# shibatch/rectdetect

Measured on AMD Instinct MI355X. Metric: 1920x1080 frames/sec, higher is better.
Workload: dtype u8/i32/f32 (bit-exact integer + IEEE f32 stencil path)

## Files before the change

rectdetect_amd/csrc/rd_k_rect.hip:

```cpp
#include <stdlib.h>
#include "rd_device.h"
#include "rd_kernels.h"
#include "rd_tidy_tile.h"
#include "rd_poly_scratch.h"
#include "rd_post_core.h"
#include <atomic>

namespace {

using namespace rd;

inline int cdiv(int a, int b) { return (a + b - 1) / b; }
const dim3 block2(64, 4);
inline dim3 grid2(int iw, int ih) { return dim3(cdiv(iw, 64), cdiv(ih, 4)); }
inline int ew_grid(int n) { int g = cdiv(n, 256 * 4); return g < 1 ? 1 : (g > 4096 ? 4096 : g); }

#define RD_XY const int x = blockIdx.x * 64 + threadIdx.x, y = blockIdx.y * 4 + rd_ty()

typedef unsigned long long u64;
__device__ __forceinline__ bitrow row_m1(const u64 *__restrict__ plane, int wpr, int y, int k, int ih) {
  if (y < 0 || y >= ih) return br(0, 0);
  const u64 *r = plane + (size_t)y * wpr + k;
  const u64 W = k > 0 ? r[-1] : 0ull, C = r[0], E = k + 1 < wpr ? r[1] : 0ull;
  return br((W >> 63) | (C << 1), (C >> 63) | (E << 1));
// ... 151 lines not shown
  const int tx = threadIdx.x, wv = rd_ty(), tid = wv * 64 + tx;
  const int x0 = rd_b.x * 64, y0 = rd_b.y * BQ_ROWS;
  const int x = x0 + tx, r0 = 8 * wv;
  const unsigned pb = (unsigned)((y0 - 4 + r0) * iw + x);
  unsigned eh[8];
  uint32_t q[8], qh;
  const int sr = tid >> 3, sc = (tid & 7) + ((tid & 4) << 4);
  const bool interior = x0 >= 4 && y0 >= 4 && x0 + 68 <= iw && y0 + BQ_ROWS + 4 <= ih;
  if (interior) {
#pragma unroll
    for (int j = 0; j < 8; j++) {
      const unsigned a = pb + (unsigned)((j < BQ_HR - 56 || r0 + j < BQ_HR ? j : 0) * iw);
      q[j] = atu(in, a);
      eh[j] = atu(ext, a);
    }
    qh = atu(in, (unsigned)((y0 - 4) * iw + x0 - 4) + (unsigned)__umul24(sr < BQ_HR ? sr : 0, iw) + (unsigned)sc);
#pragma unroll
    for (int j = BQ_HR - 56; j < 8; j++) if (r0 + j >= BQ_HR) { q[j] = 0u; eh[j] = 0u; }
  } else {
    bool ok[8];
    const bool cx = x < iw;
#pragma unroll
    for (int j = 0; j < 8; j++) {
      const int r = r0 + j, y = y0 - 4 + r;
      ok[j] = r < BQ_HR && y >= 0 && y < ih && cx;
      const unsigned a = ok[j] ? pb + (unsigned)(j * iw) : 0u;
      q[j] = atu(in, a);
      eh[j] = atu(ext, a);
    }
    const int xx = x0 - 4 + sc, yy = y0 - 4 + sr;
    const bool okq = sr < BQ_HR && xx >= 0 && xx < iw && yy >= 0 && yy < ih;
    qh = atu(in, okq ? (unsigned)(yy * iw + xx) : 0u);
#pragma unroll
    for (int j = 0; j < 8; j++) if (!ok[j]) { q[j] = 0u; eh[j] = 0u; }
    if (!okq) qh = 0u;
  }
  if (tid < 64) { const unsigned w = (unsigned)((tid & 7) + (tid >> 3)); rwt[tid] = w >= 1 && w <= 10 ? ((1u << 19) + w - 1u) / w : 0u; }
  char *const plb = (char *)pl;
  const unsigned hb = (unsigned)((r0 * BQ_SW + tx + 4) * 8);
  u64 cell[8];
#pragma unroll
  for (int j = 0; j < 8; j++) {
    const uint32_t v = q[j];
    cell[j] = (u64)((v & 4095u) | ((v << 4) & 0x3ff0000u)) | ((u64)(v >> 22) << 32);
    if (j < BQ_HR - 56 || r0 + j < BQ_HR) *(u64 *)(plb + hb + (unsigned)(j * BQ_SW * 8)) = cell[j];
  }
  if (sr < BQ_HR) pl[sr * BQ_SW + sc] = (u64)((qh & 4095u) | ((qh << 4) & 0x3ff0000u)) | ((u64)(qh >> 22) << 32);
  __syncthreads();
  {
    u64 v[9];
    const unsigned b = (unsigned)(((tx < BQ_HR ? tx : BQ_HR - 1) * BQ_SW + 9 * wv) * 8);
#pragma unroll
    for (int j = 0; j < 9; j++) v[j] = *(const u64 *)(plb + b + (unsigned)(8 * j));
    u64 sum = v[0];
#pragma unroll
    for (int j = 1; j < 9; j++) sum += v[j];
    tot[wv * 64 + tx] = sum;
    __syncthreads();
    u64 off = 0, ts[7];
#pragma unroll
    for (int s2 = 0; s2 < 7; s2++) ts[s2] = s2 < wv ? tot[s2 * 64 + tx] : 0;
#pragma unroll
    for (int s2 = 0; s2 < 7; s2++) off += ts[s2];
    if (tx < BQ_HR) {
#pragma unroll
      for (int j = 0; j < 9; j++) { *(u64 *)(plb + b + (unsigned)(8 * j)) = off; off += v[j]; }
      if (wv == 7) *(u64 *)(plb + b + 72u) = off;
    }
  }
  __syncthreads();
  u64 o[8], osum = 0;
#pragma unroll
  for (int j0 = 0; j0 < 8; j0 += BQ_WB) {
    u64 hi[BQ_WB], lo[BQ_WB];
    unsigned rw[BQ_WB];
#pragma unroll
    for (int u = 0; u < BQ_WB; u++) {
      const int j = j0 + u;
      const unsigned e = eh[j];
      const unsigned c = hb + (unsigned)((j < BQ_HR - 56 || r0 + j < BQ_HR ? j : 0) * BQ_SW * 8);
      hi[u] = *(const u64 *)(plb + c + (e & 0x38u));
      lo[u] = *(const u64 *)(plb + c + 8u - ((e & 7u) << 3));
      rw[u] = *(const unsigned *)((const char *)rwt + ((e & 63u) << 2));
    }
#pragma unroll
    for (int u = 0; u < BQ_WB; u++) {
      const int j = j0 + u;
      const u64 a = hi[u] - lo[u] + cell[j];
      const unsigned ax = (unsigned)a, ay = (unsigned)(a >> 32);
      o[j] = (u64)(div_small_m(ax & 0xffffu, rw[u]) | (div_small_m(ax >> 16, rw[u]) << 16)) | ((u64)div_small_m(ay, rw[u]) << 32);
      osum += o[j];
    }
  }
  tot[wv * 64 + tx] = osum;
  __syncthreads();
  const unsigned vb = (unsigned)((r0 * 64 + tx) * 8);
  {
    u64 off = 0, ts[7];
#pragma unroll
    for (int s2 = 0; s2 < 7; s2++) ts[s2] = s2 < wv ? tot[s2 * 64 + tx] : 0;
#pragma unroll
    for (int s2 = 0; s2 < 7; s2++) off += ts[s2];
#pragma unroll
    for (int j = 0; j < 8; j++) { *(u64 *)(plb + vb + (unsigned)(j * 512)) = off; off += o[j]; }
  }
  __syncthreads();
  if (x >= iw) return;
#pragma unroll
  for (int j0 = 0; j0 < 8; j0 += BQ_WB) {
    u64 hi[BQ_WB], lo[BQ_WB];
    unsigned rw[BQ_WB];
#pragma unroll
    for (int u = 0; u < BQ_WB; u++) {
      const int j = j0 + u, r = r0 + j;
      if (r < 4 || r >= BQ_ROWS + 4 || y0 - 4 + r >= ih) continue;
      const unsigned e = eh[j];
      const unsigned c = vb + (unsigned)(j * 512);
      hi[u] = *(const u64 *)(plb + c + (e & 0xe00u));
      lo[u] = *(const u64 *)(plb + c + 512u - ((e & 0x1c0u) << 3));
      rw[u] = *(const unsigned *)((const char *)rwt + ((e >> 4) & 0xfcu));
    }
#pragma unroll
    for (int u = 0; u < BQ_WB; u++) {
      const int j = j0 + u, r = r0 + j;
      if (r < 4 || r >= BQ_ROWS + 4 || y0 - 4 + r >= ih) continue;
      const u64 a = hi[u] - lo[u] + o[j];
      const unsigned ax = (unsigned)a, ay = (unsigned)(a >> 32);
      atu(out, pb + (unsigned)(j * iw)) = div_small_m(ax & 0xffffu, rw[u]) | (div_small_m(ax >> 16, rw[u]) << 12) | (div_small_m(ay, rw[u]) << 22);
    }
  }
}

__device__ __forceinline__ uint32_t quantize_plab(uint32_t v, int n0, int n1, int n2) {
  float L, a, b;
  unpack_lab(v, L, a, b);
  return pack_lab(roundf(L * n0) / (float)n0, roundf(a * n1) / (float)n1, roundf(b * n2) / (float)n2);
}

__device__ __attribute__((aligned(16))) uint16_t g_quant24[4096 + 1024];
__global__ void k_quant24_lut() {
  const int i = blockIdx.x * blockDim.x + threadIdx.x;
  if (i < 4096) g_quant24[i] = (uint16_t)(quantize_plab((uint32_t)i, 24, 24, 24) & 4095u);
  else if (i < 5120) g_quant24[i] = (uint16_t)((quantize_plab((uint32_t)(i - 4096) << 12, 24, 24, 24) >> 12) & 1023u);
}

#ifndef DS_ROWS
#define DS_ROWS 30
#endif
#define DS_P 66
#define DS_R (DS_ROWS + 2)
#define DS_RW (DS_R / 4)
static_assert(DS_R % 4 == 0 && 2 * DS_R <= 256 && DS_R <= 64, "rows by four waves; one halo cell per thread; a list entry is row << 6 | column in 16 bits");
template <int QN>
__global__ __launch_bounds__(256) void k_despeckle(uint32_t *__restrict__ out, const uint32_t *__restrict__ in, const float *__restrict__ edge, int iw, int ih, size_t zs, int gdim) {
  const rd_tile rd_b = rd_block_tile(gdim);
  if (rd_b.x < 0) return;
  RD_ZSHIFTZ(rd_b.z, zs, out, in, edge);
  __shared__ uint32_t tq[DS_R * DS_P];
  __shared__ uint8_t tf[DS_R * DS_P];
  __shared__ uint16_t list[4][64 * DS_RW];
  __shared__ int nlist[4];
  __shared__ uint32_t qlut[QN == 24 ? 2560 : 1];
  const int tx = threadIdx.x, wv = rd_ty(), tid = wv * 64 + tx;
  const int x0 = rd_b.x * 64, y0 = rd_b.y * DS_ROWS;
  const bool colin = x0 + tx < iw;
  const unsigned cx = (unsigned)(x0 + (colin ? tx : 0));
  uint32_t v[DS_RW + 1];
  float e[DS_RW + 1];
#pragma unroll
  for (int k = 0; k < DS_RW; k++) {
    const int y = y0 - 1 + wv + 4 * k, yc = y < 0 ? 0 : (y >= ih ? ih - 1 : y);
    const unsigned a = (unsigned)(yc * iw) + cx;
    v[k] = atu(in, a);
    e[k] = atu(edge, a);
  }
  const int hs = tid >> 1, hc = (tid & 1) * (DS_P - 1);
  const int hx = x0 - 1 + hc, hy = y0 - 1 + hs;
  const bool hok = hs < DS_R && hx >= 0 && hx < iw && hy >= 0 && hy < ih;
  {
    const unsigned a = hok ? (unsigned)(hy * iw + hx) : 0u;
    v[DS_RW] = atu(in, a);
    e[DS_RW] = atu(edge, a);
  }
  if (QN == 24) {
    uint32_t w[10];
#pragma unroll
    for (int i = 0; i < 10; i++) w[i] = atu((const uint32_t *)g_quant24, (unsigned)(tid + 256 * i));
#pragma unroll
    for (int i = 0; i < 10; i++) qlut[tid + 256 * i] = w[i];
    __syncthreads();
  }
  auto quant = [&](uint32_t c) -> uint32_t {
    if (QN == 24) {
      const uint16_t *q16 = (const uint16_t *)qlut;
      return (uint32_t)q16[c & 4095u] | ((uint32_t)q16[4096 + ((c >> 12) & 1023u)] << 12) | ((uint32_t)q16[4096 + (c >> 22)] << 22);
    }
    return QN > 0 ? quantize_plab(c, QN, QN, QN) : c;
  };
#pragma unroll
  for (int k = 0; k <= DS_RW; k++) v[k] = quant(v[k]);
  int nhot = 0;
#pragma unroll
  for (int k = 0; k < DS_RW; k++) {
    const int s = wv + 4 * k, y = y0 - 1 + s;
    const bool ok = colin && y >= 0 && y < ih, mine = ok && s >= 1 && s <= DS_ROWS;
    const uint32_t qv = v[k];
    const bool hot = !(e[k] < 1e-6f), skip = e[k] >= 1e-6f;
    const int i = s * DS_P + tx + 1;
    tq[i] = qv;
    tf[i] = ok && !skip ? 0 : 1;
    if (mine && !hot) atu(out, (unsigned)(y * iw + x0 + tx)) = qv;
    const unsigned long long m = __builtin_amdgcn_ballot_w64(mine && hot);
    if (m) {
      if (mine && hot) list[wv][nhot + (int)__builtin_amdgcn_mbcnt_hi((unsigned)(m >> 32), __builtin_amdgcn_mbcnt_lo((unsigned)m, 0u))] = (uint16_t)((s << 6) | tx);
      nhot += __popcll(m);
    }
  }
  if (hs < DS_R) {
    const int i = hs * DS_P + hc;
    tq[i] = v[DS_RW];
    tf[i] = hok && !(e[DS_RW] >= 1e-6f) ? 0 : 1;
  }
  if (tx == 0) nlist[wv] = nhot;
  __syncthreads();
  const int n1 = nlist[0], n2 = n1 + nlist[1], n3 = n2 + nlist[2], n = n3 + nlist[3];
  for (int j = tid; j < n; j += 256) {
    const int w = (j >= n1) + (j >= n2) + (j >= n3);
    const int en = list[w][j - (w == 0 ? 0 : (w == 1 ? n1 : (w == 2 ? n2 : n3)))];
    const int s = en >> 6, c = en & 63;
    const int i = s * DS_P + c + 1;
    uint32_t r = tq[i];
    float dist = 1e+10f, l0, a0, b0;
    unpack_lab(r, l0, a0, b0);
#pragma unroll
    for (int k = 0; k < 9; k++) {
      const int q = i + (k / 3 - 1) * DS_P + k % 3 - 1;
      if (tf[q]) continue;
      float l1, a1, b1;
      const uint32_t v1 = tq[q];
      unpack_lab(v1, l1, a1, b1);
      const float dx = l1 - l0, dy = a1 - a0, dz = b1 - b0;
      const float d = sqrtf(dx * dx + dy * dy + dz * dz);
      if (d < dist) { r = v1; dist = d; }
    }
    atu(out, (unsigned)((y0 + s - 1) * iw + x0 + c)) = r;
  }
}

template <int DX>
__device__ __forceinline__ unsigned long long mm_shift(unsigned long long w0, unsigned long long w1, unsigned long long w2) {
  if (DX == 0) return w1;
  if (DX > 0) return (w1 >> DX) | (w2 << (64 - DX));
  return (w1 << -DX) | (w0 >> (64 + DX));
}
template <int DY, int LO, int HI, int DX = -8>
__device__ __forceinline__ unsigned long long mm_row(unsigned long long w0, unsigned long long w1, unsigned long long w2) {
  unsigned long long r = 0;
  if (DX * DX + DY * DY >= LO && DX * DX + DY * DY < HI) r = mm_shift<DX>(w0, w1, w2);
  if constexpr (DX < 8) r |= mm_row<DY, LO, HI, DX + 1>(w0, w1, w2);
  return r;
}
template <int DY>
__device__ __forceinline__ void mm_rows(const unsigned long long *sb, int r, unsigned long long &A, unsigned long long &B, unsigned long long &C) {
  const unsigned long long *row = sb + (r + 8 + DY) * 6;
  const unsigned long long a0 = row[0], a1 = row[1], a2 = row[2], e0 = row[3], e1 = row[4], e2 = row[5];
  constexpr int ADY = DY < 0 ? -DY : DY;
  if (ADY * ADY < 36) A |= mm_row<ADY, 16, 36>(a0, a1, a2);
  if (ADY * ADY < 64) B |= mm_row<ADY, 0, 64>(e0, e1, e2);
  if (ADY * ADY < 16) C |= mm_row<ADY, 0, 16>(a0 & ~e0, a1 & ~e1, a2 & ~e2);
  if constexpr (DY < 8) mm_rows<DY + 1>(sb, r, A, B, C);
}

#define MM_ROWS 64
__global__ __launch_bounds__(256) void k_mm_gather(unsigned long long *__restrict__ out, const unsigned long long *__restrict__ bits, int iw, int ih, int wpr, size_t zs) {
  RD_ZSHIFT(zs, out, bits);
  __shared__ unsigned long long sb[(MM_ROWS + 16) * 6];
  const int k = blockIdx.x;
  const int y0 = blockIdx.y * MM_ROWS;
  const int tid = rd_ty() * 64 + threadIdx.x;
  for (int t = tid; t < (MM_ROWS + 16) * 6; t += 256) {
    const int r = t / 6, j = t % 6;
    const int yy = y0 - 8 + r, kk = k - 1 + j % 3;
    unsigned long long v = 0ull;
    if (yy >= 0 && yy < ih && kk >= 0 && kk < wpr) v = bits[((size_t)yy * wpr + kk) * 2 + j / 3];
    sb[t] = v;
  }
  __syncthreads();
  if (tid < MM_ROWS && y0 + tid < ih) {
    unsigned long long A = 0, B = 0, C = 0;
    mm_rows<-8>(sb, tid, A, B, C);
    const int left = iw - 64 * k;
    out[(size_t)(y0 + tid) * wpr + k] = A & ~B & ~C & (left >= 64 ? ~0ull : ((1ull << left) - 1ull));
  }
}

#define RR_NFLAGS (RD_REGION_STATUS_AT + 32)
static_assert(RD_REGION_STATUS_AT >= RD_REGION_MAX_LAUNCHES && RR_NFLAGS <= 256, "k_region_init clears the flag words with one block of 256 threads");
#ifndef RI_ROWS
#define RI_ROWS 32
#endif
#define RI_H 10
#define RI_RW (64 + RI_H + 2)
#define RI_RH (RI_ROWS + RI_H + 2)
#define RI_NC (RI_RW * RI_RH)
__global__ __launch_bounds__(256) void k_region_init(int *__restrict__ A, int *__restrict__ B, u64 *__restrict__ allow, const int *__restrict__ pix, const u64 *__restrict__ mask,
                                                     const u64 *__restrict__ edge, int iw, int ih, int wpr, int *__restrict__ flags, int *__restrict__ size_out, size_t zs, int gdim) {
  const rd_tile rd_b = rd_block_tile(gdim);
  if (rd_b.x < 0) return;
  RD_ZSHIFTZ(rd_b.z, zs, A, B, allow, pix, mask, edge, flags, size_out);
  __shared__ u64 sm[(RI_ROWS + 2) * 2];
  __shared__ u64 se[(RI_ROWS + 3) * 3];
  __shared__ int col[RI_NC];
  __shared__ short lnk[RI_NC];
  __shared__ short prop[RI_NC];
  __shared__ unsigned char alw[RI_NC];
  const int tid = rd_ty() * 64 + threadIdx.x;
  if (rd_b.x == 0 && rd_b.y == 0 && tid < RR_NFLAGS) flags[tid] = tid == 0 ? 1 : 0;
  const int gx0 = rd_b.x * 64 - RI_H, gy0 = rd_b.y * RI_ROWS - RI_H;
  {
    constexpr int NR = (RI_RH + 3) / 4, NS = (RI_RH * 16 + 255) / 256;
    const int wv = rd_ty(), lx = threadIdx.x;
    int v[NR + NS];
    bool ok[NR + NS];
    u64 wm = 0, we = 0;
    bool okm = false, oke = false;
    {
      const int k = rd_b.x, yb0 = rd_b.y * RI_ROWS;
      { const int r = tid >> 1, kk = k + (tid & 1), yy = yb0 + r; okm = tid < (RI_ROWS + 2) * 2 && yy < ih && kk < wpr; wm = mask[okm ? (size_t)yy * wpr + kk : 0]; }
      { const int r = tid / 3, kk = k - 1 + tid % 3, yy = yb0 - 1 + r; oke = tid < (RI_ROWS + 3) * 3 && yy >= 0 && yy < ih && kk >= 0 && kk < wpr; we = edge[oke ? (size_t)yy * wpr + kk : 0]; }
    }
    const int gxl = gx0 + lx;
    const bool cok = gxl >= 0 && gxl < iw;
#pragma unroll
    for (int i = 0; i < NR; i++) {
      const int r = wv + 4 * i, gy = gy0 + r;
      ok[i] = r < RI_RH && gy >= 0 && gy < ih && cok;
      v[i] = atu(pix, ok[i] ? (unsigned)(gy * iw + gxl) : 0u);
    }
#pragma unroll
    for (int j = 0; j < NS; j++) {
      const int t = tid + 256 * j, r = t >> 4, c = 64 + (t & 15);
      const int gx = gx0 + c, gy = gy0 + r;
      ok[NR + j] = r < RI_RH && c < RI_RW && gx < iw && gy >= 0 && gy < ih;
      v[NR + j] = atu(pix, ok[NR + j] ? (unsigned)(gy * iw + gx) : 0u);
    }
#pragma unroll
    for (int i = 0; i < NR; i++) {
      const int r = wv + 4 * i;
      if (r < RI_RH) { col[r * RI_RW + lx] = v[i]; lnk[r * RI_RW + lx] = ok[i] ? 0 : -1; }
    }
#pragma unroll
    for (int j = 0; j < NS; j++) {
      const int t = tid + 256 * j, r = t >> 4, c = 64 + (t & 15);
      if (r < RI_RH && c < RI_RW) { col[r * RI_RW + c] = v[NR + j]; lnk[r * RI_RW + c] = ok[NR + j] ? 0 : -1; }
    }
    if (tid < (RI_ROWS + 2) * 2) sm[tid] = okm ? wm : 0ull;
    if (tid < (RI_ROWS + 3) * 3) se[tid] = oke ? we : 0ull;
  }
  constexpr int MW = 64 + 2, MH = RI_ROWS + 2, MN = MW * MH;
  __syncthreads();
  (void)MN;
  {
    auto cell = [&](int cy, int cx) {
      const int gx = gx0 + RI_H + cx, gy = gy0 + RI_H + cy;
      const unsigned mbit = (unsigned)(sm[cy * 2 + (cx >> 6)] >> (cx & 63)) & 1u, ebit = (unsigned)(se[(cy + 1) * 3 + 1 + (cx >> 6)] >> (cx & 63)) & 1u;
      alw[(RI_H + cy) * RI_RW + RI_H + cx] = (unsigned char)((gx < iw && gy < ih) ? (mbit | (ebit ? 0u : 2u)) : 0u);
    };
    for (int cy = rd_ty(); cy < MH; cy += 4) cell(cy, (int)threadIdx.x);
    if (tid < 2 * MH) cell(tid >> 1, 64 + (tid & 1));
    static_assert(MW == 66, "two columns beyond the lanes");
  }
  {
    auto cell = [&](int cy, int cx) {
      const int t = cy * RI_RW + cx;
      if (lnk[t] < 0) return;
      const int gx = gx0 + cx, gy = gy0 + cy;
      int l = t;
      if (gy > 0 && cy > 0 && col[t] == col[t - RI_RW]) l = t - RI_RW;
      else if (gx > 0 && cx > 0 && col[t] == col[t - 1]) l = t - 1;
      lnk[t] = (short)l;
    };
    for (int cy = rd_ty(); cy < RI_RH; cy += 4) cell(cy, (int)threadIdx.x);
    for (int t = tid; t < RI_RH * 16; t += 256) { const int c = 64 + (t & 15); if (c < RI_RW) cell(t >> 4, c); }
  }
  __syncthreads();
  constexpr int NPR = (RI_ROWS + 1 + 3) / 4, NP = NPR + 1;
  const int wvp = rd_ty(), lxp = threadIdx.x;
  int pcx[NP], pcy[NP];
  bool pin[NP];
#pragma unroll
  for (int i = 0; i < NP; i++) {
    pcy[i] = i < NPR ? wvp + 4 * i : tid;
    pcx[i] = i < NPR ? lxp : 64;
    pin[i] = pcy[i] < RI_ROWS + 1;
  }
  unsigned char anew[NP];
#pragma unroll
  for (int i = 0; i < NP; i++) {
    unsigned a = 0;
    if (pin[i]) {
      const int cx = RI_H + pcx[i], cy = RI_H + pcy[i], c = cy * RI_RW + cx;
      const int gx = gx0 + cx, gy = gy0 + cy;
      if (gx > 0 && gy > 0 && gx < iw - 1 && gy < ih - 1) {
        const unsigned b0 = alw[c];
        const bool any = (b0 & 1) != 0, z0 = (b0 & 2) != 0;
        const int v = col[c];
        if ((v == col[c - RI_RW] || any) && z0) a |= 1;
        if ((v == col[c - 1] || any) && z0) a |= 2;
        if ((v == col[c + 1] || any) && (alw[c + 1] & 2)) a |= 4;
        if ((v == col[c + RI_RW] || any) && (alw[c + RI_RW] & 2)) a |= 8;
        a |= 16;
      }
    }
    anew[i] = (unsigned char)a;
  }
  __syncthreads();
#pragma unroll
  for (int i = 0; i < NP; i++)
    if (pin[i]) alw[(RI_H + pcy[i]) * RI_RW + RI_H + pcx[i]] = anew[i];
  __syncthreads();
  {
    int m[NP], og[NP], cc[NP];
    bool act[NP];
#pragma unroll
    for (int i = 0; i < NP; i++) {
      const bool in = pin[i];
      const int c = in ? (RI_H + pcy[i]) * RI_RW + RI_H + pcx[i] : RI_H * RI_RW + RI_H;
      const unsigned a = in ? alw[c] : 0u;
      cc[i] = in ? c : -1;
      act[i] = (a & 16) != 0;
      og[i] = act[i] ? lnk[c] : RI_H * RI_RW + RI_H;
      int mm = og[i];
      if (a & 1) { const int s = lnk[c - RI_RW]; mm = s < mm ? s : mm; }
      if (a & 2) { const int s = lnk[c - 1]; mm = s < mm ? s : mm; }
      if (a & 4) { const int s = lnk[c + 1]; mm = s < mm ? s : mm; }
      if (a & 8) { const int s = lnk[c + RI_RW]; mm = s < mm ? s : mm; }
      m[i] = mm;
    }
#pragma unroll
    for (int j = 0; j < 8; j++)
#pragma unroll
      for (int i = 0; i < NP; i++) m[i] = lnk[m[i]];
#pragma unroll
    for (int i = 0; i < NP; i++) if (cc[i] >= 0) prop[cc[i]] = (short)((act[i] && m[i] != og[i]) ? m[i] : 0x7fff);
  }
  __syncthreads();
  const int x = rd_b.x * 64 + threadIdx.x;
  if (x >= iw) return;
  for (int r = rd_ty(); r < RI_ROWS; r += 4) {
    const int y = rd_b.y * RI_ROWS + r;
    if (y >= ih) break;
    const int c = (r + RI_H) * RI_RW + threadIdx.x + RI_H, p = y * iw + x;
    int l = lnk[c];
    const int g0 = prop[c];
    l = g0 < l ? g0 : l;
    if (x + 1 < iw && lnk[c + 1] == c) { const int g1 = prop[c + 1]; l = g1 < l ? g1 : l; }
    if (y + 1 < ih && lnk[c + RI_RW] == c) { const int g2 = prop[c + RI_RW]; l = g2 < l ? g2 : l; }
    const int w = ((gy0 + l / RI_RW) * iw + gx0 + l % RI_RW) << 3;
    A[p] = w;
    B[p] = w;
    if (size_out) {
      int j = 0;
      const int b = threadIdx.x;
      if (x > 0 && y > 0 && x < iw - 1 && y < ih - 1 && ((se[(r + 1) * 3 + 1] >> b) & 1ull)) {
        int cnt = 0;
#pragma unroll
        for (int dr = 0; dr < 3; dr++) {
          const u64 *w = &se[(r + dr) * 3];
          const unsigned v = b == 0 ? (((unsigned)w[1] & 3u) << 1) | (unsigned)(w[0] >> 63) : (b == 63 ? ((unsigned)(w[1] >> 62) & 3u) | (((unsigned)w[2] & 1u) << 2) : (unsigned)(w[1] >> (b - 1)) & 7u);
          cnt += __popc(v);
        }
        j = cnt == 1 ? 0 : cnt;
      }
      size_out[p] = j;
    }
  }
  static_assert(RI_ROWS == 32, "four waves, eight rows each");
  {
    const int r0 = rd_ty() * 8, y0 = rd_b.y * RI_ROWS + r0;
    if (y0 < ih) {
      u64 w = 0;
#pragma unroll
      for (int k = 0; k < 8; k++) w |= (u64)((y0 + k < ih) ? alw[(r0 + k + RI_H) * RI_RW + threadIdx.x + RI_H] : 0) << (8 * k);
      allow[(size_t)(y0 >> 3) * iw + x] = w;
    }
  }
}

#ifndef RR_PX
#define RR_PX 8
#endif
#ifndef RR_TY
#define RR_TY 4
#endif
#define RR_MBITS 3
#ifndef RR_DEEP
#define RR_DEEP 3
#endif
__device__ __forceinline__ int rr_label(const int *X, unsigned q) { return at32(X, q) >> RR_MBITS; }
template <int PHASE, bool INNER>
__device__ __forceinline__ void rr_tile(const int *X, int *Y, const u64 *__restrict__ allow, int iw, int ih, int *flags, int round, int bx, int by, int *hk, int *hv, int *tmin) {
  const int tid = rd_ty() * 64 + threadIdx.x;
  constexpr bool near = PHASE == 1;
  const int mark = 1 + round % 7, mark_prev = round > 0 ? 1 + (round - 1) % 7 : 8;
  const int lx = (int)threadIdx.x, ly = rd_ty() * RR_PX;
  const int yb = by * (RR_TY * RR_PX) + ly;
  const int x0 = bx * 64, x = x0 + lx;
  const unsigned rowb = (unsigned)iw << 2;
  unsigned pb[RR_PX];
  int og[RR_PX], g[RR_PX], nx[RR_PX], w0[RR_PX];
  unsigned a[RR_PX];
  bool valid[RR_PX], act[RR_PX], todo[RR_PX];
  {
    int l[RR_PX][5];
    int ed[RR_PX];
    static_assert(RR_PX == 8, "the allow bytes of a thread's 8 rows are one word (k_region_init)");
    if (INNER) {
      const unsigned tb = (unsigned)(yb * iw + x0) << 2;
      const u64 aw = atu(allow, (unsigned)((yb >> 3) * iw + x0) + (unsigned)lx);
      const unsigned b0 = tb + ((unsigned)lx << 2), e0 = tb + (lx < 32 ? 0u - 4u : 256u);
#pragma unroll
      for (int k = 0; k < RR_PX; k++) {
        valid[k] = true;
        pb[k] = b0 + (unsigned)k * rowb;
        a[k] = (unsigned)(aw >> (8 * k)) & 0xffu;
        l[k][0] = atb(X, pb[k]);
      }
      l[0][1] = atb(X, pb[0] - rowb);
      l[RR_PX - 1][4] = atb(X, pb[RR_PX - 1] + rowb);
#pragma unroll
      for (int k = 0; k < RR_PX; k++) ed[k] = atb(X, e0 + (unsigned)k * rowb);
    } else {
      const bool colin = x < iw && yb < ih;
      const u64 aw = allow[colin ? (size_t)(yb >> 3) * iw + x : 0];
#pragma unroll
      for (int k = 0; k < RR_PX; k++) {
        const int y = yb + k;
        valid[k] = x < iw && y < ih;
        pb[k] = valid[k] ? (unsigned)(y * iw + x) << 2 : 0u;
        a[k] = valid[k] ? (unsigned)(aw >> (8 * k)) & 0xffu : 0u;
        l[k][0] = atb(X, pb[k]);
      }
      l[0][1] = atb(X, (valid[0] && yb > 0) ? pb[0] - rowb : pb[0]);
      l[RR_PX - 1][4] = atb(X, (valid[RR_PX - 1] && yb + RR_PX - 1 < ih - 1) ? pb[RR_PX - 1] + rowb : pb[RR_PX - 1]);
      const int xe = lx < 32 ? x0 - 1 : x0 + 64;
#pragma unroll
      for (int k = 0; k < RR_PX; k++) {
        const int y = yb + k;
        ed[k] = atb(X, (y < ih && xe >= 0 && xe < iw) ? (unsigned)(y * iw + xe) << 2 : pb[k]);
      }
    }
#pragma unroll
    for (int k = 0; k < RR_PX; k++) {
      l[k][2] = __builtin_amdgcn_update_dpp(ed[k], l[k][0], 0x138, 0xf, 0xf, false);
      l[k][3] = __builtin_amdgcn_update_dpp(ed[k], l[k][0], 0x130, 0xf, 0xf, false);
    }
#pragma unroll
    for (int k = 0; k < RR_PX; k++) {
      if (k > 0) l[k][1] = l[k - 1][0];
      if (k < RR_PX - 1) l[k][4] = l[k + 1][0];
    }
#pragma unroll
    for (int k = 0; k < RR_PX; k++) {
      w0[k] = l[k][0];
      int m = w0[k];
#pragma unroll
      for (int c = 1; c < 5; c++) {
        const int t = __builtin_amdgcn_sbfe((int)a[k], c - 1, 1);
        const int xk = (l[k][c] & t) | (0x7fffffff & ~t);
        m = xk < m ? xk : m;
      }
      og[k] = w0[k] >> RR_MBITS;
      g[k] = m >> RR_MBITS;
      act[k] = INNER || (a[k] & 16);
    }
  }
  const float inv_iw = 1.0f / (float)iw;
#pragma unroll
  for (int k = 0; k < RR_PX; k++) {
    const int v = rr_label(X, (unsigned)g[k]);
    nx[k] = act[k] ? v : g[k];
  }
  for (int j = 1; j < 8; j++) {
    bool moving = false;
#pragma unroll
    for (int k = 0; k < RR_PX; k++) moving = moving || nx[k] != g[k];
    if (!__any(moving)) break;
#pragma unroll
    for (int k = 0; k < RR_PX; k++) { g[k] = nx[k]; nx[k] = rr_label(X, (unsigned)nx[k]); }
  }
  bool any_todo = false;
#pragma unroll
  for (int k = 0; k < RR_PX; k++) {
    g[k] = act[k] ? nx[k] : og[k];
    todo[k] = g[k] != og[k];
    const bool lag = (w0[k] & 7) == mark_prev;
    if (!near && (INNER || valid[k]) && (todo[k] || lag)) atomicMin(&atb(Y, pb[k]), (g[k] << RR_MBITS) | (todo[k] ? mark : 0));
    any_todo = any_todo || todo[k];
  }
  if (near) {
    const int origin = by * (RR_TY * RR_PX) * iw + bx * 64;
    bool out[RR_PX];
#pragma unroll
    for (int k = 0; k < RR_PX; k++) {
      const int d = og[k] - origin;
      bool inside = false;
      int cell = 0;
      if (d >= 0 && d < RR_TY * RR_PX * iw) {
        int row = (int)((float)d * inv_iw), col = d - row * iw;
        if (col < 0) { row--; col += iw; } else if (col >= iw) { row++; col -= iw; }
        inside = col < 64 && row < RR_TY * RR_PX && bx * 64 + col < iw;
        cell = row * 64 + col;
      }
      if (todo[k] && inside) atomicMin(&tmin[cell], g[k]);
      out[k] = todo[k] && !inside;
    }
#pragma unroll
    for (int k = 0; k < RR_PX; k++) { const int w = (g[k] << RR_MBITS) | mark; if (out[k]) atomicMin(&Y[og[k]], w); }
    __syncthreads();
#pragma unroll
    for (int k = 0; k < RR_PX; k++) {
      if (!INNER && !valid[k]) continue;
      const bool lag = (w0[k] & 7) == mark_prev;
      int w = (todo[k] || lag) ? ((g[k] << RR_MBITS) | (todo[k] ? mark : 0)) : 0x7fffffff;
      const int h = tmin[(ly + k) * 64 + lx];
      if (h != 0x7fffffff) { const int wh = (h << RR_MBITS) | mark; w = wh < w ? wh : w; }
      if (w != 0x7fffffff) atomicMin(&atb(Y, pb[k]), w);
    }
    if (__any(any_todo) && threadIdx.x == 0) flags[round] = 1;
    return;
  }
  auto hook = [&](int key, int val) {
    const int w = (val << RR_MBITS) | mark;
    if (w < ld_agent(&Y[key])) atomicMin(&Y[key], w);
  };
  if (__any(any_todo)) {
    bool need[RR_PX];
#pragma unroll
    for (int k = 0; k < RR_PX; k++) {
      const int pog = __builtin_amdgcn_mov_dpp(og[k], 0x138, 0xf, 0xf, true), pg = __builtin_amdgcn_mov_dpp(g[k], 0x138, 0xf, 0xf, true);
      need[k] = todo[k] && (pog != og[k] || pg != g[k]);
    }
    if (PHASE == 2) {
#pragma unroll
      for (int k = 0; k < RR_PX; k++) { const int w = (g[k] << RR_MBITS) | mark; if (need[k] && w < ld_agent(&Y[og[k]])) atomicMin(&Y[og[k]], w); }
    } else {
#pragma unroll
      for (int k = 0; k < RR_PX; k++) {
        if (!need[k]) continue;
        unsigned h = ((unsigned)og[k] * 2654435761u) >> 23;
        int probes = 0;
        for (;;) {
          const int kprev = atomicCAS(&hk[h], -1, og[k]);
          if (kprev == -1 || kprev == og[k]) { atomicMin(&hv[h], g[k]); break; }
          h = (h + 1) & 511;
          if (++probes == 16) { hook(og[k], g[k]); break; }
        }
      }
    }
    if (threadIdx.x == 0) flags[round] = 1;
  }
  if (PHASE != 3) return;
  __syncthreads();
  for (int t = tid; t < 512; t += 64 * RR_TY) {
    const int key = hk[t];
    if (key != -1) hook(key, hv[t]);
  }
}

template <int PHASE>
__global__ __launch_bounds__(64 * RR_TY) void k_region_round(int *X, int *Y, const u64 *__restrict__ allow, int iw, int ih, int *flags, int round, size_t zs, int gdim) {
  const int z = rd_block_frame(gdim);
  if (round > 0 && *(const int *)((const char *)(flags + (round - 1)) + (size_t)z * zs) == 0) return;
  const rd_tile rd_b = rd_block_tile_of(gdim, z);
  if (rd_b.x < 0) return;
  const int bx = rd_b.x, by = rd_b.y;
  RD_ZSHIFTZ(rd_b.z, zs, X, Y, allow, flags);
  __shared__ int hk[PHASE == 3 ? 512 : 1], hv[PHASE == 3 ? 512 : 1];
  __shared__ int tmin[PHASE == 1 ? 64 * RR_TY * RR_PX : 1];
  const int tid = rd_ty() * 64 + threadIdx.x;
  if (PHASE == 3) for (int t = tid; t < 512; t += 64 * RR_TY) { hk[t] = -1; hv[t] = 0x7fffffff; }
  if (PHASE == 1) for (int t = tid; t < 64 * RR_TY * RR_PX; t += 64 * RR_TY) tmin[t] = 0x7fffffff;
  if (PHASE != 2) __syncthreads();
  const bool inner = bx > 0 && by > 0 && bx * 64 + 65 <= iw && by * (RR_TY * RR_PX) + RR_TY * RR_PX + 1 <= ih;
  if (inner) rr_tile<PHASE, true>(X, Y, allow, iw, ih, flags, round, bx, by, hk, hv, tmin);
  else rr_tile<PHASE, false>(X, Y, allow, iw, ih, flags, round, bx, by, hk, hv, tmin);
}

#define RS_T 1024
#ifndef RS_PER_THREAD
#define RS_PER_THREAD 32
#endif
__device__ __forceinline__ void rs_accum(int *keys, int *vals, int *out, int label, int cnt) {
  unsigned h = ((unsigned)label * 2654435761u) >> 22;
  int probes = 0;
  for (;;) {
    const int kprev = atomicCAS(&keys[h], -1, label);
    if (kprev == -1 || kprev == label) { atomicAdd(&vals[h], cnt); return; }
    h = (h + 1) & (RS_T - 1);
    if (++probes == 32) { atomicAdd(&out[label], cnt); return; }
  }
}

__global__ __launch_bounds__(256) void k_region_size(int *out, int *__restrict__ label, int n, int *zero_me, int marked, size_t zs) {
  RD_ZSHIFT(zs, out, label, zero_me);
  if (zero_me && blockIdx.x == 0 && threadIdx.x == 0) *zero_me = 0;
  __shared__ int keys[RS_T], vals[RS_T];
  for (int i = threadIdx.x; i < RS_T; i += 256) { keys[i] = -1; vals[i] = 0; }
  __syncthreads();
  const int begin = blockIdx.x * 256 * RS_PER_THREAD;
  int lks[RS_PER_THREAD];
#pragma unroll
  for (int k = 0; k < RS_PER_THREAD; k++) {
    const int i = begin + k * 256 + threadIdx.x;
    lks[k] = i < n ? label[i] : -1;
  }
  if (marked) {
#pragma unroll
    for (int k = 0; k < RS_PER_THREAD; k++) {
      const int i = begin + k * 256 + threadIdx.x;
      if (i < n) { lks[k] >>= RR_MBITS; label[i] = lks[k]; }
    }
  }
#pragma unroll
  for (int k = 0; k < RS_PER_THREAD; k++) {
    const int lk = lks[k];
    const int l0 = __shfl(lk, 0);
    if (__all(lk == l0)) {
      if ((threadIdx.x & 63) == 0 && l0 != -1) rs_accum(keys, vals, out, l0, 64);
      continue;
    }
    const int lane = threadIdx.x & 63;
    const int prev = __shfl_up(lk, 1);
    const bool start = lane == 0 || prev != lk;
    const unsigned long long after = __ballot(start) & ~((2ull << lane) - 1ull);
    if (start && lk != -1) rs_accum(keys, vals, out, lk, (after ? __ffsll((long long)after) - 1 : 64) - lane);
  }
  __syncthreads();
  for (int i = threadIdx.x; i < RS_T; i += 256)
    if (keys[i] != -1 && vals[i] != 0) atomicAdd(&out[keys[i]], vals[i]);
}

__device__ __forceinline__ int despeckle2_pick(const int *__restrict__ cur, const int *__restrict__ old, const int *__restrict__ size, int l0, int x, int y, int iw, int ih) {
  const int p0 = y * iw + x;
  int lab[9], sz[9];
  bool ok[9];
#pragma unroll
  for (int k = 0; k < 9; k++) {
    const int xx = k % 3 - 1, yy = k / 3 - 1;
    ok[k] = !(x + xx < 0 || x + xx >= iw || y + yy < 0 || y + yy >= ih);
    const int p1 = ok[k] ? p0 + yy * iw + xx : p0;
    lab[k] = k < 4 ? cur[p1] : old[p1];
  }
#pragma unroll
  for (int k = 0; k < 9; k++) sz[k] = size[lab[k]];
  int res = l0, maxSize = 0;
#pragma unroll
  for (int k = 0; k < 9; k++) if (ok[k] && sz[k] > maxSize) { maxSize = sz[k]; res = lab[k]; }
  return res;
}

#define D2_ROWS 32
__global__ __launch_bounds__(256) void k_despeckle2_first(int *__restrict__ nxt, int *__restrict__ other, int *__restrict__ stamp, int *__restrict__ list, int *count,
                                                           const int *__restrict__ old, const int *__restrict__ size, int thre, int iw, int ih) {
  __shared__ int loc[64 * D2_ROWS];
  __shared__ int nloc, base;
  if (threadIdx.x == 0 && rd_ty() == 0) {
    nloc = 0;
    if (blockIdx.x == 0 && blockIdx.y == 0) count[1] = count[2] = 0;
  }
  __syncthreads();
  const int x = blockIdx.x * 64 + threadIdx.x;
  int l0s[D2_ROWS / 4], szs[D2_ROWS / 4];
#pragma unroll
  for (int k = 0; k < D2_ROWS / 4; k++) {
    const int y = blockIdx.y * D2_ROWS + rd_ty() + 4 * k;
    l0s[k] = old[(x < iw && y < ih) ? y * iw + x : 0];
  }
#pragma unroll
  for (int k = 0; k < D2_ROWS / 4; k++) szs[k] = size[l0s[k]];
#pragma unroll
  for (int k = 0; k < D2_ROWS / 4; k++) {
    const int r = rd_ty() + 4 * k;
    const int y = blockIdx.y * D2_ROWS + r;
    const bool inside = x < iw && y < ih;
    const int p0 = y * iw + x;
    bool small = false;
    if (inside) {
      const int l0 = l0s[k];
// ... 903 lines not shown
```

Measured before the change: 3486.

## Restructure region init tile into packed shared cells with inner/border specialization

Rewrites k_region_init around one packed byte-addressed shared array that holds link words and allow/flag bytes, replacing separate col/lnk/prop/alw arrays. The same-colour left-neighbour test now uses DPP lane shifts, mask and edge bits come through readlane and inverse_ballot, and allow bits are computed in registers. This drops two barriers and an LDS round trip. Interior tiles take a template path with no bounds checks, and the kernel requests 8 waves per EU. In exchange it adds heavy register and bit-packing complexity, with a risk of spills or divergence on border tiles.

```diff
diff --git a/rectdetect_amd/csrc/rd_k_rect.hip b/rectdetect_amd/csrc/rd_k_rect.hip
--- a/rectdetect_amd/csrc/rd_k_rect.hip
+++ b/rectdetect_amd/csrc/rd_k_rect.hip
@@ -477,189 +477,235 @@
 #define RI_H 10
 #define RI_RW (64 + RI_H + 2)
 #define RI_RH (RI_ROWS + RI_H + 2)
-#define RI_NC (RI_RW * RI_RH)
-__global__ __launch_bounds__(256) void k_region_init(int *__restrict__ A, int *__restrict__ B, u64 *__restrict__ allow, const int *__restrict__ pix, const u64 *__restrict__ mask,
+#define RI_PB 256
+#define RI_BY 160
+#define RI_PP 66
+#define RI_MR (RI_RH / 4)
+#define RI_SR 3
+static_assert(RI_ROWS == 32, "four waves, eight rows each: a thread's allow bytes are one word of k_region_round");
+static_assert(RI_RH % 4 == 0 && 16 * RI_SR >= RI_RH && 2 * RI_RW <= RI_BY && RI_BY + RI_RW <= RI_PB && RI_RH * RI_PB < 0x7fff, "staging layout; a cell number stays below the 'no proposal' word");
+__device__ __forceinline__ unsigned ri_link(const unsigned char *cells, unsigned o) { return *(const unsigned short *)(cells + o); }
+template <int BIT> __device__ __forceinline__ unsigned ri_barred(unsigned a) { return ~(unsigned)((int)(a << (31 - BIT)) >> 31); }
+template <bool INNER>
+__device__ __forceinline__ void ri_tile(int *__restrict__ A, int *__restrict__ B, u64 *__restrict__ allow, const int *__restrict__ pix, const u64 *__restrict__ mask, const u64 *__restrict__ edge,
+                                        int iw, int ih, int wpr, int *__restrict__ size_out, int bx, int by, unsigned char *cells, unsigned short *prop, unsigned *sx) {
+  const int wv = rd_ty(), lx = (int)threadIdx.x, tid = wv * 64 + lx;
+  const int x0 = bx * 64, y0 = by * RI_ROWS, gx0 = x0 - RI_H, gy0 = y0 - RI_H;
+  {
+    int v[RI_MR + 1], s[RI_SR + 1];
+    unsigned sm[RI_SR], se[RI_SR];
+    bool sok[RI_SR];
+    const int r0 = wv * RI_MR;
+    const int gxl = gx0 + lx, cxl = INNER ? gxl : clampi(gxl, 0, iw - 1);
+#pragma unroll
+    for (int i = 0; i <= RI_MR; i++) {
+      const int r = r0 - 1 + i;
+      int gy = gy0 + (r < 0 ? 0 : r);
+      if (!INNER) gy = clampi(gy, 0, ih - 1);
+      v[i] = atu(pix, (unsigned)(gy * iw) + (unsigned)cxl);
+    }
+    unsigned wbits;
+    {
+      const int i = lx & 15, r = r0 + (i < RI_MR ? i : RI_MR - 1), yy = y0 + (r < RI_H ? 0 : r - RI_H);
+      const bool okw = INNER || yy < ih;
+      const unsigned *pl = (const unsigned *)((lx & 16) ? edge : mask);
+      wbits = atu(pl, (unsigned)((okw ? yy : 0) * wpr + bx) * 2u + (unsigned)(lx >> 5));
+      if (!okw) wbits = 0u;
+    }
+    const int sj = tid & 15, sr0 = (tid >> 4) * RI_SR;
+    const int sgx = gx0 + 60 + sj, cxs = INNER ? sgx : (sgx < iw ? sgx : iw - 1);
+#pragma unroll
+    for (int i = 0; i <= RI_SR; i++) {
+      int gy = gy0 + clampi(sr0 - 1 + i, 0, RI_RH - 1);
+      if (!INNER) gy = clampi(gy, 0, ih - 1);
+      s[i] = atu(pix, (unsigned)(gy * iw + cxs));
+    }
+    const int stc = 50 + sj, skk = bx + (stc >> 6), sbit = stc & 31;
+#pragma unroll
+    for (int i = 0; i < RI_SR; i++) {
+      const int yy = y0 + clampi(sr0 + i, RI_H, RI_RH - 1) - RI_H;
+      sok[i] = INNER || (yy < ih && skk < wpr);
+      const unsigned a = sok[i] ? (unsigned)(yy * wpr + skk) * 2u + (unsigned)((stc >> 5) & 1) : 0u;
+      sm[i] = atu((const unsigned *)mask, a);
+      se[i] = atu((const unsigned *)edge, a);
+    }
+    u64 j1;
+    unsigned j0, j2;
+    {
+      const int yy = y0 - 1 + tid;
+      const bool ok1 = tid < RI_ROWS + 2 && (INNER || (yy >= 0 && yy < ih)), ok0 = ok1 && (INNER || bx > 0), ok2 = ok1 && (INNER || bx + 1 < wpr);
+      const unsigned a = (unsigned)((ok1 ? yy : 0) * wpr + bx);
+      j0 = atu((const unsigned *)edge, ok0 ? 2u * a - 1u : 0u);
+      j1 = atu(edge, ok1 ? a : 0u);
+      j2 = atu((const unsigned *)edge, ok2 ? 2u * a + 2u : 0u);
+      if (!ok0) j0 = 0u;
+      if (!ok1) j1 = 0ull;
+      if (!ok2) j2 = 0u;
+    }
+    const unsigned mo = (unsigned)(r0 * RI_PB + 2 * lx), mb0 = (unsigned)(r0 * RI_PB + RI_BY + lx);
+    const bool colok = INNER || (gxl >= 0 && gxl < iw), colproc = INNER || (gxl > 0 && gxl < iw - 1);
+#pragma unroll
+    for (int i = 0; i < RI_MR; i++) {
+      const int r = r0 + i, gy = gy0 + r;
+      const int me = v[i + 1];
+      const int lf = __builtin_amdgcn_update_dpp(me, me, 0x138, 0xf, 0xf, false);
+      bool su = me == v[i] && r > 0, sl = me == lf && lx > 0;
+      const u64 wm = (u64)(unsigned)__builtin_amdgcn_readlane((int)wbits, i) | ((u64)(unsigned)__builtin_amdgcn_readlane((int)wbits, 32 + i) << 32);
+      const u64 we = (u64)(unsigned)__builtin_amdgcn_readlane((int)wbits, 16 + i) | ((u64)(unsigned)__builtin_amdgcn_readlane((int)wbits, 48 + i) << 32);
+      bool mb = __builtin_amdgcn_inverse_ballot_w64(wm << RI_H), ns = !__builtin_amdgcn_inverse_ballot_w64(we << RI_H);
+      bool proc = true;
+      if (!INNER) {
+        const bool ok = colok && gy >= 0 && gy < ih;
+        su = su && ok && gy > 0;
+        sl = sl && ok && gxl > 0;
+        mb = mb && ok;
+        ns = ns && ok;
+        proc = colproc && gy > 0 && gy < ih - 1;
+      }
+      const unsigned o = mo + (unsigned)(i * RI_PB);
+      *(unsigned short *)(cells + o) = (unsigned short)(o - (su ? (unsigned)RI_PB : (sl ? 2u : 0u)));
+      (cells + mb0)[i * RI_PB] = (unsigned char)((su ? 1u : 0u) | (sl ? 2u : 0u) | (mb ? 4u : 0u) | (ns ? 8u : 0u) | (proc ? 16u : 0u));
+    }
+#pragma unroll
+    for (int i = 0; i < RI_SR; i++) {
+      const int r = sr0 + i, gy = gy0 + r;
+      const int me = s[i + 1];
+      const int lf = __builtin_amdgcn_update_dpp(me, me, 0x111, 0xf, 0xf, false);
+      bool su = me == s[i] && r > 0, sl = me == lf;
+      bool mb = sok[i] && ((sm[i] >> sbit) & 1u), ns = !(sok[i] && ((se[i] >> sbit) & 1u));
+      bool proc = true;
+      if (!INNER) {
+        const bool ok = sgx < iw && gy >= 0 && gy < ih;
+        su = su && ok && gy > 0;
+        sl = sl && ok;
+        mb = mb && ok;
+        ns = ns && ok;
+        proc = sgx < iw - 1 && gy > 0 && gy < ih - 1;
+      }
+      if (sj >= 4 && r < RI_RH) {
+        const unsigned o = (unsigned)(r * RI_PB + 2 * (60 + sj));
+        *(unsigned short *)(cells + o) = (unsigned short)(su ? o - RI_PB : (sl ? o - 2u : o));
+        cells[r * RI_PB + RI_BY + 60 + sj] = (unsigned char)((su ? 1u : 0u) | (sl ? 2u : 0u) | (mb ? 4u : 0u) | (ns ? 8u : 0u) | (proc ? 16u : 0u));
+      }
+    }
+    if (tid < RI_ROWS + 2) {
+      sx[tid * 3] = ((unsigned)j1 << 1) | (j0 >> 31);
+      sx[tid * 3 + 1] = (unsigned)(j1 >> 31);
+      sx[tid * 3 + 2] = (unsigned)(j1 >> 63) | ((j2 & 1u) << 1);
+    }
+  }
+  __syncthreads();
+  const int C = RI_H + lx, R0 = RI_H + 8 * wv;
+  const unsigned ob = (unsigned)(R0 * RI_PB + 2 * C);
+  const bool ev = wv == 0 || (wv == 1 && lx <= RI_ROWS);
+  const int er = wv == 0 ? RI_H + RI_ROWS : RI_H + (ev ? lx : 0), ec = wv == 0 ? C : RI_H + 64;
+  const unsigned eo = (unsigned)(er * RI_PB + 2 * ec);
+  unsigned t[8];
+  unsigned aw[2] = {0u, 0u};
+  {
+    unsigned bo[9], br[8], lc[10], ll[8], lr[8], be[3], le[5], al[9];
+#pragma unroll
+    for (int k = 0; k < 9; k++) bo[k] = cells[(R0 + k) * RI_PB + RI_BY + C];
+#pragma unroll
+    for (int k = 0; k < 8; k++) br[k] = cells[(R0 + k) * RI_PB + RI_BY + C + 1];
+    be[0] = cells[er * RI_PB + RI_BY + ec];
+    be[1] = cells[er * RI_PB + RI_BY + ec + 1];
+    be[2] = cells[(er + 1) * RI_PB + RI_BY + ec];
+    auto allowed = [](unsigned b, unsigned r, unsigned d) -> unsigned {
+      const unsigned any = (b >> 2) & 1u, ns = (b >> 3) & 1u;
+      unsigned a = ((b | (0u - any)) & (0u - ns) & 3u) | ((((r >> 1) | any) & (r >> 3) & 1u) << 2) | (((d | any) & (d >> 3) & 1u) << 3) | 16u;
+      if (!INNER) a = (b & 16u) ? a : 0u;
+      return a;
+    };
+#pragma unroll
+    for (int k = 0; k < 8; k++) {
+      al[k] = allowed(bo[k], br[k], bo[k + 1]) | ((((br[k] >> 1) & ~br[k]) & 1u) << 5) | ((bo[k + 1] & 1u) << 6);
+      asm volatile("" : "+v"(al[k]));
+      aw[k >> 2] |= al[k] << (8 * (k & 3));
+    }
+    al[8] = allowed(be[0], be[1], be[2]);
+    asm volatile("" : "+v"(al[8]));
+#pragma unroll
+    for (int j = 0; j < 10; j++) lc[j] = ri_link(cells, ob + (unsigned)((j - 1) * RI_PB));
+#pragma unroll
+    for (int k = 0; k < 8; k++) { ll[k] = ri_link(cells, ob + (unsigned)(k * RI_PB) - 2u); lr[k] = ri_link(cells, ob + (unsigned)(k * RI_PB) + 2u); }
+    le[0] = ri_link(cells, eo);
+    le[1] = ri_link(cells, eo - RI_PB);
+    le[2] = ri_link(cells, eo - 2u);
+    le[3] = ri_link(cells, eo + 2u);
+    le[4] = ri_link(cells, eo + RI_PB);
+    auto least = [](unsigned a, unsigned self, unsigned up, unsigned left, unsigned right, unsigned down) -> unsigned {
+      const unsigned m0 = min(self, min(up | ri_barred<0>(a), left | ri_barred<1>(a)));
+      return min(m0, min(right | ri_barred<2>(a), down | ri_barred<3>(a)));
+    };
+    unsigned m[9];
+    bool act[9];
+#pragma unroll
+    for (int k = 0; k < 8; k++) {
+      act[k] = INNER || (al[k] & 16u);
+      m[k] = least(al[k], lc[k + 1], lc[k], ll[k], lr[k], lc[k + 2]);
+    }
+    act[8] = INNER || (al[8] & 16u);
+    m[8] = least(al[8], le[0], le[1], le[2], le[3], le[4]);
+#pragma unroll
+    for (int j = 0; j < 8; j++)
+#pragma unroll
+      for (int k = 0; k < 9; k++) m[k] = ri_link(cells, m[k]);
+#pragma unroll
+    for (int k = 0; k < 8; k++) {
+      const unsigned pv = (act[k] && m[k] != lc[k + 1]) ? m[k] : 0x7fffu;
+      prop[(8 * wv + k) * RI_PP + lx] = (unsigned short)pv;
+      t[k] = min(lc[k + 1], pv);
+    }
+    if (ev) prop[(er - RI_H) * RI_PP + ec - RI_H] = (unsigned short)((act[8] && m[8] != le[0]) ? m[8] : 0x7fffu);
+  }
+  __syncthreads();
+  const int x = x0 + lx, yw = y0 + 8 * wv;
+  const bool colin = INNER || x < iw;
+  unsigned pr[9];
+#pragma unroll
+  for (int k = 0; k < 8; k++) pr[k] = prop[(8 * wv + k) * RI_PP + lx + 1];
+  pr[8] = prop[(8 * wv + 8) * RI_PP + lx];
+  unsigned win = 0;
+  if (size_out) {
+    const unsigned *q = sx + 8 * wv * 3 + (lx >> 5);
+#pragma unroll
+    for (int i = 0; i < 10; i++) win |= (__builtin_amdgcn_alignbit(q[i * 3 + 1], q[i * 3], (unsigned)lx & 31u) & 7u) << (3 * i);
+  }
+#pragma unroll
+  for (int k = 0; k < 8; k++) {
+    const unsigned ab = aw[k >> 2] >> (8 * (k & 3));
+    unsigned l = t[k];
+    l = (ab & 32u) ? min(l, pr[k]) : l;
+    l = (ab & 64u) ? min(l, k < 7 ? t[k + 1] : pr[8]) : l;
+    const int w = ((gy0 + (int)(l >> 8)) * iw + gx0 + (int)((l >> 1) & 127u)) << 3;
+    const int y = yw + k;
+    const unsigned p = (unsigned)(y * iw + x);
+    if (colin && (INNER || y < ih)) {
+      atu(A, p) = w;
+      atu(B, p) = w;
+      if (size_out) {
+        const unsigned b9 = (win >> (3 * k)) & 0x1ffu;
+        const int cnt = __popc(b9);
+        atu(size_out, p) = ((b9 & 16u) && cnt != 1 && (INNER || (ab & 16u))) ? cnt : 0;
+      }
+    }
+  }
+  if (colin && (INNER || yw < ih)) atu(allow, (unsigned)((yw >> 3) * iw + x)) = ((u64)(aw[1] & 0x1f1f1f1fu) << 32) | (u64)(aw[0] & 0x1f1f1f1fu);
+}
+__global__ __launch_bounds__(256) __attribute__((amdgpu_waves_per_eu(8))) void k_region_init(int *__restrict__ A, int *__restrict__ B, u64 *__restrict__ allow, const int *__restrict__ pix, const u64 *__restrict__ mask,
                                                      const u64 *__restrict__ edge, int iw, int ih, int wpr, int *__restrict__ flags, int *__restrict__ size_out, size_t zs, int gdim) {
   const rd_tile rd_b = rd_block_tile(gdim);
   if (rd_b.x < 0) return;
   RD_ZSHIFTZ(rd_b.z, zs, A, B, allow, pix, mask, edge, flags, size_out);
-  __shared__ u64 sm[(RI_ROWS + 2) * 2];
-  __shared__ u64 se[(RI_ROWS + 3) * 3];
-  __shared__ int col[RI_NC];
-  __shared__ short lnk[RI_NC];
-  __shared__ short prop[RI_NC];
-  __shared__ unsigned char alw[RI_NC];
-  const int tid = rd_ty() * 64 + threadIdx.x;
+  __shared__ __attribute__((aligned(16))) unsigned char cells[RI_RH * RI_PB];
+  __shared__ unsigned short prop[(RI_ROWS + 1) * RI_PP];
+  __shared__ unsigned sx[(RI_ROWS + 2) * 3];
+  const int tid = rd_ty() * 64 + (int)threadIdx.x;
   if (rd_b.x == 0 && rd_b.y == 0 && tid < RR_NFLAGS) flags[tid] = tid == 0 ? 1 : 0;
-  const int gx0 = rd_b.x * 64 - RI_H, gy0 = rd_b.y * RI_ROWS - RI_H;
-  {
-    constexpr int NR = (RI_RH + 3) / 4, NS = (RI_RH * 16 + 255) / 256;
-    const int wv = rd_ty(), lx = threadIdx.x;
-    int v[NR + NS];
-    bool ok[NR + NS];
-    u64 wm = 0, we = 0;
-    bool okm = false, oke = false;
-    {
-      const int k = rd_b.x, yb0 = rd_b.y * RI_ROWS;
-      { const int r = tid >> 1, kk = k + (tid & 1), yy = yb0 + r; okm = tid < (RI_ROWS + 2) * 2 && yy < ih && kk < wpr; wm = mask[okm ? (size_t)yy * wpr + kk : 0]; }
-      { const int r = tid / 3, kk = k - 1 + tid % 3, yy = yb0 - 1 + r; oke = tid < (RI_ROWS + 3) * 3 && yy >= 0 && yy < ih && kk >= 0 && kk < wpr; we = edge[oke ? (size_t)yy * wpr + kk : 0]; }
-    }
-    const int gxl = gx0 + lx;
-    const bool cok = gxl >= 0 && gxl < iw;
-#pragma unroll
-    for (int i = 0; i < NR; i++) {
-      const int r = wv + 4 * i, gy = gy0 + r;
-      ok[i] = r < RI_RH && gy >= 0 && gy < ih && cok;
-      v[i] = atu(pix, ok[i] ? (unsigned)(gy * iw + gxl) : 0u);
-    }
-#pragma unroll
-    for (int j = 0; j < NS; j++) {
-      const int t = tid + 256 * j, r = t >> 4, c = 64 + (t & 15);
-      const int gx = gx0 + c, gy = gy0 + r;
-      ok[NR + j] = r < RI_RH && c < RI_RW && gx < iw && gy >= 0 && gy < ih;
-      v[NR + j] = atu(pix, ok[NR + j] ? (unsigned)(gy * iw + gx) : 0u);
-    }
-#pragma unroll
-    for (int i = 0; i < NR; i++) {
-      const int r = wv + 4 * i;
-      if (r < RI_RH) { col[r * RI_RW + lx] = v[i]; lnk[r * RI_RW + lx] = ok[i] ? 0 : -1; }
-    }
-#pragma unroll
-    for (int j = 0; j < NS; j++) {
-      const int t = tid + 256 * j, r = t >> 4, c = 64 + (t & 15);
-      if (r < RI_RH && c < RI_RW) { col[r * RI_RW + c] = v[NR + j]; lnk[r * RI_RW + c] = ok[NR + j] ? 0 : -1; }
-    }
-    if (tid < (RI_ROWS + 2) * 2) sm[tid] = okm ? wm : 0ull;
-    if (tid < (RI_ROWS + 3) * 3) se[tid] = oke ? we : 0ull;
-  }
-  constexpr int MW = 64 + 2, MH = RI_ROWS + 2, MN = MW * MH;
-  __syncthreads();
-  (void)MN;
-  {
-    auto cell = [&](int cy, int cx) {
-      const int gx = gx0 + RI_H + cx, gy = gy0 + RI_H + cy;
-      const unsigned mbit = (unsigned)(sm[cy * 2 + (cx >> 6)] >> (cx & 63)) & 1u, ebit = (unsigned)(se[(cy + 1) * 3 + 1 + (cx >> 6)] >> (cx & 63)) & 1u;
-      alw[(RI_H + cy) * RI_RW + RI_H + cx] = (unsigned char)((gx < iw && gy < ih) ? (mbit | (ebit ? 0u : 2u)) : 0u);
-    };
-    for (int cy = rd_ty(); cy < MH; cy += 4) cell(cy, (int)threadIdx.x);
-    if (tid < 2 * MH) cell(tid >> 1, 64 + (tid & 1));
-    static_assert(MW == 66, "two columns beyond the lanes");
-  }
-  {
-    auto cell = [&](int cy, int cx) {
-      const int t = cy * RI_RW + cx;
-      if (lnk[t] < 0) return;
-      const int gx = gx0 + cx, gy = gy0 + cy;
-      int l = t;
-      if (gy > 0 && cy > 0 && col[t] == col[t - RI_RW]) l = t - RI_RW;
-      else if (gx > 0 && cx > 0 && col[t] == col[t - 1]) l = t - 1;
-      lnk[t] = (short)l;
-    };
-    for (int cy = rd_ty(); cy < RI_RH; cy += 4) cell(cy, (int)threadIdx.x);
-    for (int t = tid; t < RI_RH * 16; t += 256) { const int c = 64 + (t & 15); if (c < RI_RW) cell(t >> 4, c); }
-  }
-  __syncthreads();
-  constexpr int NPR = (RI_ROWS + 1 + 3) / 4, NP = NPR + 1;
-  const int wvp = rd_ty(), lxp = threadIdx.x;
-  int pcx[NP], pcy[NP];
-  bool pin[NP];
-#pragma unroll
-  for (int i = 0; i < NP; i++) {
-    pcy[i] = i < NPR ? wvp + 4 * i : tid;
-    pcx[i] = i < NPR ? lxp : 64;
-    pin[i] = pcy[i] < RI_ROWS + 1;
-  }
-  unsigned char anew[NP];
-#pragma unroll
-  for (int i = 0; i < NP; i++) {
-    unsigned a = 0;
-    if (pin[i]) {
-      const int cx = RI_H + pcx[i], cy = RI_H + pcy[i], c = cy * RI_RW + cx;
-      const int gx = gx0 + cx, gy = gy0 + cy;
-      if (gx > 0 && gy > 0 && gx < iw - 1 && gy < ih - 1) {
-        const unsigned b0 = alw[c];
-        const bool any = (b0 & 1) != 0, z0 = (b0 & 2) != 0;
-        const int v = col[c];
-        if ((v == col[c - RI_RW] || any) && z0) a |= 1;
-        if ((v == col[c - 1] || any) && z0) a |= 2;
-        if ((v == col[c + 1] || any) && (alw[c + 1] & 2)) a |= 4;
-        if ((v == col[c + RI_RW] || any) && (alw[c + RI_RW] & 2)) a |= 8;
-        a |= 16;
-      }
-    }
-    anew[i] = (unsigned char)a;
-  }
-  __syncthreads();
-#pragma unroll
-  for (int i = 0; i < NP; i++)
-    if (pin[i]) alw[(RI_H + pcy[i]) * RI_RW + RI_H + pcx[i]] = anew[i];
-  __syncthreads();
-  {
-    int m[NP], og[NP], cc[NP];
-    bool act[NP];
-#pragma unroll
-    for (int i = 0; i < NP; i++) {
-      const bool in = pin[i];
-      const int c = in ? (RI_H + pcy[i]) * RI_RW + RI_H + pcx[i] : RI_H * RI_RW + RI_H;
-      const unsigned a = in ? alw[c] : 0u;
-      cc[i] = in ? c : -1;
-      act[i] = (a & 16) != 0;
-      og[i] = act[i] ? lnk[c] : RI_H * RI_RW + RI_H;
-      int mm = og[i];
-      if (a & 1) { const int s = lnk[c - RI_RW]; mm = s < mm ? s : mm; }
-      if (a & 2) { const int s = lnk[c - 1]; mm = s < mm ? s : mm; }
-      if (a & 4) { const int s = lnk[c + 1]; mm = s < mm ? s : mm; }
-      if (a & 8) { const int s = lnk[c + RI_RW]; mm = s < mm ? s : mm; }
-      m[i] = mm;
-    }
-#pragma unroll
-    for (int j = 0; j < 8; j++)
-#pragma unroll
-      for (int i = 0; i < NP; i++) m[i] = lnk[m[i]];
-#pragma unroll
-    for (int i = 0; i < NP; i++) if (cc[i] >= 0) prop[cc[i]] = (short)((act[i] && m[i] != og[i]) ? m[i] : 0x7fff);
-  }
-  __syncthreads();
-  const int x = rd_b.x * 64 + threadIdx.x;
-  if (x >= iw) return;
-  for (int r = rd_ty(); r < RI_ROWS; r += 4) {
-    const int y = rd_b.y * RI_ROWS + r;
-    if (y >= ih) break;
-    const int c = (r + RI_H) * RI_RW + threadIdx.x + RI_H, p = y * iw + x;
-    int l = lnk[c];
-    const int g0 = prop[c];
-    l = g0 < l ? g0 : l;
-    if (x + 1 < iw && lnk[c + 1] == c) { const int g1 = prop[c + 1]; l = g1 < l ? g1 : l; }
-    if (y + 1 < ih && lnk[c + RI_RW] == c) { const int g2 = prop[c + RI_RW]; l = g2 < l ? g2 : l; }
-    const int w = ((gy0 + l / RI_RW) * iw + gx0 + l % RI_RW) << 3;
-    A[p] = w;
-    B[p] = w;
-    if (size_out) {
-      int j = 0;
-      const int b = threadIdx.x;
-      if (x > 0 && y > 0 && x < iw - 1 && y < ih - 1 && ((se[(r + 1) * 3 + 1] >> b) & 1ull)) {
-        int cnt = 0;
-#pragma unroll
-        for (int dr = 0; dr < 3; dr++) {
-          const u64 *w = &se[(r + dr) * 3];
-          const unsigned v = b == 0 ? (((unsigned)w[1] & 3u) << 1) | (unsigned)(w[0] >> 63) : (b == 63 ? ((unsigned)(w[1] >> 62) & 3u) | (((unsigned)w[2] & 1u) << 2) : (unsigned)(w[1] >> (b - 1)) & 7u);
-          cnt += __popc(v);
-        }
-        j = cnt == 1 ? 0 : cnt;
-      }
-      size_out[p] = j;
-    }
-  }
-  static_assert(RI_ROWS == 32, "four waves, eight rows each");
-  {
-    const int r0 = rd_ty() * 8, y0 = rd_b.y * RI_ROWS + r0;
-    if (y0 < ih) {
-      u64 w = 0;
-#pragma unroll
-      for (int k = 0; k < 8; k++) w |= (u64)((y0 + k < ih) ? alw[(r0 + k + RI_H) * RI_RW + threadIdx.x + RI_H] : 0) << (8 * k);
-      allow[(size_t)(y0 >> 3) * iw + x] = w;
-    }
-  }
+  const bool inner = rd_b.x >= 1 && rd_b.y >= 1 && 64 * rd_b.x + 66 <= iw && RI_ROWS * rd_b.y + RI_ROWS + 2 <= ih;
+  if (inner) ri_tile<true>(A, B, allow, pix, mask, edge, iw, ih, wpr, size_out, rd_b.x, rd_b.y, cells, prop, sx);
+  else ri_tile<false>(A, B, allow, pix, mask, edge, iw, ih, wpr, size_out, rd_b.x, rd_b.y, cells, prop, sx);
 }
 
 #ifndef RR_PX
```

New measurement: 3496 (median of 6 runs). No clear change (+0.3%).
